# Autonomous-Drone-Racing-Lab/Efficient-Path-Planner

Hardware: AMD Instinct MI355X
Metric: validity checks/sec + full plan ms/track, 1/2/4/8 MI355X vs CPU ref (higher is better)
Workload: dtype f64; 1 GPU; C2: 1 track, 8 gates, 64 OBBs, 1,048,576 sampled states per step; obbs=64, can_pass_gate=False, parallelism=replicas x1 (independent samplers), process_group=solo, launch=hip graph of the K steps

## Files before the change

### efficient-path-planner_amd/csrc/collision_common.h

```cpp
#pragma once
#include <hip/hip_runtime.h>

#include <algorithm>
#include <cstdlib>
#include <mutex>
#include <set>
#include <string>

#include "epp_internal.h"

namespace epp {
SmallWorld small_world(const epp_world* w);
epp_status note_record_reader(const epp_world* w, const SmallWorld& sw, hipStream_t st);

constexpr int64_t kSmallStates = 4096;
constexpr int64_t kSmallMotions = 1024;
constexpr int kSmallMaxObbs = 256;
bool small_states(const SmallWorld& sw, int64_t n);
bool small_motions(const SmallWorld& sw, int64_t n);
epp_status launch_states_small(const SmallWorld& sw, bool mindist, const double* xyz, int64_t n, int32_t can_pass,
                               double md, uint8_t* valid, int32_t* compact_idx, int64_t* n_valid, hipStream_t st,
                               uint32_t* done = nullptr, uint32_t seq = 0);
epp_status launch_motions_small(const SmallWorld& sw, int32_t mode, const double* s1, const double* s2, int64_t n,
                                int32_t can_pass, uint8_t* valid, hipStream_t st, uint32_t* done = nullptr,
// ... 341 lines not shown
    const double tx = fillb ? rr[F_HX] : rr[F_HX] + r, ty = fillb ? rr[F_HY] : rr[F_HY] + r,
                 tz = fillb ? rr[F_HZ] : rr[F_HZ] + r;
    clip(c * ax + sn * ay, c * d[0] + sn * d[1], -tx, tx);
    clip(c * ay - sn * ax, c * d[1] - sn * d[0], -ty, ty);
    clip(ps[2] - rr[F_CZ], d[2], -tz, tz);
    int k0 = 33, k1 = 0;
    if (t0 <= t1) {
        k0 = max(1, (int)ceil(32.0 * t0));
        k1 = min(32, (int)floor(32.0 * t1));
    }
    bool hit = false;
    for (int k = k0; k <= k1 && !hit; ++k) {
        const double t = (double)k / 32.0;
        const double qx = ps[0] + (pe[0] - ps[0]) * t;
        const double qy = ps[1] + (pe[1] - ps[1]) * t;
        const double qz = ps[2] + (pe[2] - ps[2]) * t;
        hit = rec_hit<false>(rr, rg, ro, qx, qy, qz, cp, 0.0);
    }
    return hit;
}

template <bool MINDIST>
__device__ __forceinline__ bool states_exact_rec(const unsigned char* sbase, uint32_t lists_off, uint32_t ids_off,
                                                 double rg, double ro, double px, double py, double pz, uint32_t cls,
                                                 int can_pass, double md) {
    const double* recs = reinterpret_cast<const double*>(sbase);
    const uint32_t h = reinterpret_cast<const uint32_t*>(sbase + lists_off)[cls];
    const uint16_t* ids = reinterpret_cast<const uint16_t*>(sbase + ids_off) + (h >> 12);
    const uint32_t cnt = h & 4095u;
    bool hit = false;
    for (uint32_t j = 0; j < cnt; ++j)
        hit |= rec_hit<MINDIST>(recs + (size_t)ids[j] * kRecDoubles, rg, ro, px, py, pz, can_pass != 0, md);
    return hit;
}


__device__ __forceinline__ bool rec_ray_hit(const double* rec, const double s[3], const double e[3], double r) {
    double f[kRecDoubles];
#pragma unroll
    for (int k = 0; k <= F_HZ; ++k) f[k] = rec[k];
    f[R_META] = rec[R_META];
    const uint32_t m = (uint32_t)__double_as_longlong(f[R_META]);
    const bool fill = (m & META_FILLING) != 0u;
    const double c = f[F_COS], sn = f[F_SIN];
    const double cx = f[F_CX], cy = f[F_CY], cz = f[F_CZ];
    const double h[3] = {f[F_HX], f[F_HY], f[F_HZ]};
    const double ph0 = fill ? h[0] : h[0] + r, ph1 = fill ? h[1] : h[1] + r, ph2 = fill ? h[2] : h[2] + r;
    double ls[3], ld[3];
    bool end_hit;
    {
        const double dx = s[0] - cx, dy = s[1] - cy, dz = s[2] - cz;
        ls[0] = c * dx + sn * dy;
        ls[1] = c * dy - sn * dx;
        ls[2] = dz;
        const double ex = e[0] - cx, ey = e[1] - cy, ez = e[2] - cz;
// ... 90 lines not shown
```

### efficient-path-planner_amd/csrc/epp_internal.h

```cpp
#pragma once
#include <math.h>
#include <stdint.h>

#include <mutex>
#include <shared_mutex>
#include <string>
#include <vector>

#include <hip/hip_runtime_api.h>

#include "epp.h"

namespace epp {
epp_status generate_trajectory_into(const double* wp, int32_t n_wp, const double* times, double v_max,
                                    double a_max, double dt, double t0, const double v0[3], const double a0[3],
                                    double* (*alloc)(void*, int64_t), void* ctx, int64_t* n_rows);
struct FusedCheck {
    const epp_world* world;
    const double* xyz;
    int64_t n;
    double min_distance;
    uint8_t* valid;
};
epp_status check_and_generate_into(const FusedCheck* chk, const double* wp, int32_t n_wp, const double* times,
// ... 44 lines not shown
           o_query = 0, o_ids32 = 0, o_rows32 = 0, o_rows16 = 0, o_ev = 0, o_mark = 0, o_map = 0, o_nstat = 0,
           o_need = 0, dev_bytes = 0;
    size_t h_seg = 0, h_hdr = 0, h_slot = 0, h_rows = 0, h_need = 0, h_done = 0, host_bytes = 0;
    int32_t done_n = 0;
};
PlanBatchLayout plan_batch_layout(int32_t S, int64_t ns, int32_t k, PlanSeg* segs);
void plan_batch_trace_print();
epp_status plan_batch_launch(const epp_world* world, int32_t can_pass_gate, const double lo[3], const double hi[3],
                             const PlanBatchLayout& L, void* dev, void* host, uint32_t seq, void* stream);
}

namespace epp {

enum Field : int {
    F_LOX = 0, F_LOY, F_LOZ, F_HIX, F_HIY, F_HIZ,
    F_CX, F_CY, F_CZ,
    F_COS, F_SIN,
    F_HX, F_HY, F_HZ,
    EPP_NF
};

constexpr int kRecDoubles = 17;
constexpr int R_META = 16;

constexpr size_t kListMaxLen = 4095;
constexpr size_t kStageBudget = 64 * 1024;

constexpr uint32_t META_FILLING = 1u;
constexpr uint32_t META_GATE = 2u;
constexpr int kMaxGridAxis = 255;

struct WorldView {
    const unsigned char* blob;
    uint32_t blob_bytes;
    int32_t n_obb;
    int32_t n_pad;
    int32_t nx, ny, nz;
    uint32_t front_bytes;
    uint32_t off_cell_mask;
    uint32_t off_cell_start;
    uint32_t off_cell_obb;
    uint32_t off_meta;
    uint32_t off_soa;
    double gx0, gy0, gz0;
    double gx1, gy1, gz1;
    double icx, icy, icz;
    float ofx, ofy, ofz;
    float i4x, i4y, i4z;
    float limx, limy, limz;
    float fmaxx, fmaxy, fmaxz;
    double r_gate, r_obst;
    uint32_t off_aos;
    uint32_t off_lists;
    uint32_t off_ids;
    uint32_t n_lists;
    uint32_t off_bitmap;
    uint32_t bm_words;
    uint32_t off_cls8;
    uint32_t cls8_bytes;
    int32_t bnx, bny, bnz;
    float bofx, bofy, bofz;
    float bix, biy, biz;
    uint32_t off_slab;
    int32_t slab_n;
    int32_t slab_log;
    int32_t slab_w;
    int32_t tile_n;
    uint32_t tile_words;
    float sofx, sofy, sofz;
    float six, siy, siz;
};

constexpr int kSlabMaxWords = 32;
constexpr size_t kSlabBudget = 40 * 1024;
constexpr size_t kSlabBudgetMax = 64 * 1024;
constexpr size_t kMotionsLdsFree = 150 * 1024 - 16 * (256 * 4 + 64);
#if defined(__HIPCC__)
// ... 88 lines not shown
```

### efficient-path-planner_amd/csrc/states.hip

```cpp
#include "collision_common.h"

namespace epp {
namespace {

template <int STAGE, bool MINDIST, bool ALIGNED>
__global__ __launch_bounds__(kBlock) void k_states(WorldView w, const double* __restrict__ xyz,
                                                   int64_t n, int can_pass, double md,
                                                   uint8_t* __restrict__ valid,
                                                   int32_t* __restrict__ compact_idx,
                                                   unsigned long long* __restrict__ n_valid,
                                                   uint32_t stage_bytes) {
    extern __shared__ __attribute__((aligned(16))) unsigned char lds[];
    const int lane = threadIdx.x & 63;
    const int64_t groups = n / 4;
    const int64_t stride = (int64_t)gridDim.x * kBlock;
    auto load = [&](int64_t grp, double (&dst)[12]) {
        grp = grp < groups ? grp : groups - 1;
        if (ALIGNED) {
            const double2* q = reinterpret_cast<const double2*>(xyz + 12 * grp);
#pragma unroll
            for (int k = 0; k < 6; ++k) {
                const double2 t = q[k];
                dst[2 * k] = t.x;
                dst[2 * k + 1] = t.y;
// ... 155 lines not shown
    extern __shared__ __attribute__((aligned(16))) unsigned char lds_blob[];
    const int lane = threadIdx.x & 63;
    const int wave = __builtin_amdgcn_readfirstlane(threadIdx.x >> 6);
    BmParams bp;
    bp.cls = (gptr_u16)(wv->blob + wv->off_bitmap);
    bp.ox = wv->bofx; bp.oy = wv->bofy; bp.oz = wv->bofz;
    bp.ix = wv->bix; bp.iy = wv->biy; bp.iz = wv->biz;
    bp.nx = (uint32_t)wv->bnx; bp.ny = (uint32_t)wv->bny; bp.nz = (uint32_t)wv->bnz;
    bp.sentinel = wv->bm_words;
    const uint32_t stride = gridDim.x * kBlock4;
    uint32_t it = blockIdx.x * kBlock4 + threadIdx.x;
    double v[6];
    auto load = [&](uint32_t i) {
        i = i < items ? i : items - 1;
        const double2* p = reinterpret_cast<const double2*>(xyz) + 3 * (size_t)i;
#pragma unroll
        for (int k = 0; k < 3; ++k) {
            const double2 t = p[k];
            v[2 * k] = t.x;
            v[2 * k + 1] = t.y;
        }
    };
    if (items > 0) load(it);
    const uint32_t lists_off = wv->off_lists - wv->off_aos, ids_off = wv->off_ids - wv->off_aos;
    const double rg = wv->r_gate, ro = wv->r_obst;
    const unsigned char* xbase;
    if (STAGE) {
        stage_copy(lds_blob, wv->blob + wv->off_aos, stage_bytes, kBlock4);
        xbase = lds_blob;
    } else {
        xbase = wv->blob + wv->off_aos;
    }
    for (uint32_t i0 = blockIdx.x * kBlock4; i0 < items; i0 += stride, it += stride) {
        if (i0 != blockIdx.x * kBlock4) load(it);
        const bool live = it < items;
        const uint32_t c0 = bp.cls[cls_index(bp, v[0], v[1], v[2])];
        const uint32_t c1 = bp.cls[cls_index(bp, v[3], v[4], v[5])];
        const bool n0 = live & (c0 != 0u), n1 = live & (c1 != 0u);
        const unsigned long long b0 = __ballot(n0), b1 = __ballot(n1);
        const uint32_t t0 = (uint32_t)__popcll(b0), tw = t0 + (uint32_t)__popcll(b1);
        if (lane == 0) q.wcnt[wave] = tw;
        __syncthreads();
        uint32_t off = 0, T = 0;
        for (int w = 0; w < wave; ++w) off += q.wcnt[w];
        T = off;
        for (int w = wave; w < kBlock4 / 64; ++w) T += q.wcnt[w];
        uint32_t hits = 0;
        if (T > 0) {
            const uint32_t p0 = off + lanes_below(b0), p1 = off + t0 + lanes_below(b1);
            if (n0) {
                q.x[p0] = v[0];
                q.y[p0] = v[1];
                q.z[p0] = v[2];
                q.cls[p0] = (uint16_t)c0;
            }
            if (n1) {
                q.x[p1] = v[3];
                q.y[p1] = v[4];
                q.z[p1] = v[5];
                q.cls[p1] = (uint16_t)c1;
            }
            __syncthreads();
            for (uint32_t e = threadIdx.x; e < T; e += kBlock4)
                q.hit[e] = states_exact_rec<MINDIST>(xbase, lists_off, ids_off, rg, ro, q.x[e], q.y[e], q.z[e], q.cls[e],
                                                     can_pass, md)
                               ? 1
                               : 0;
            __syncthreads();
            hits = (n0 && q.hit[p0] ? 1u : 0u) | (n1 && q.hit[p1] ? 2u : 0u);
        }
        const uint32_t fl = live ? (~hits & 3u) : 0u;
        if (live) *reinterpret_cast<uint16_t*>(valid + 2 * (size_t)it) = (uint16_t)((fl & 1u) | ((fl & 2u) << 7));
        if (COMPACT) {
            const uint32_t c = (uint32_t)__popc(fl);
            uint32_t ctot;
            const uint32_t cex = wave_excl_scan(c, lane, ctot);
            unsigned long long wbase = 0;
            if (lane == 0 && ctot) wbase = atomicAdd(n_valid, (unsigned long long)ctot);
            wbase = __shfl(wbase, 0, 64);
            uint64_t p = wbase + cex;
            if (fl & 1u) compact_idx[p++] = (int32_t)(2 * (size_t)it);
            if (fl & 2u) compact_idx[p] = (int32_t)(2 * (size_t)it + 1);
        }
    }
    if (STAGE && items == 0) __syncthreads();
    if (blockIdx.x == 0 && threadIdx.x == 0 && (n & 1)) {
        const int64_t i = n - 1;
        const double px = xyz[3 * i], py = xyz[3 * i + 1], pz = xyz[3 * i + 2];
        const uint32_t c = bp.cls[cls_index(bp, px, py, pz)];
        const bool ok = !(c != 0u && states_exact_rec<MINDIST>(xbase, lists_off, ids_off, rg, ro, px, py, pz, c, can_pass, md));
        valid[i] = ok ? 1 : 0;
        if (COMPACT && ok) compact_idx[atomicAdd(n_valid, 1ull)] = (int32_t)i;
    }
}

struct WaveQueue5 {
    double x[64], y[64], z[64];
    uint32_t hdr[64];
};
template <int BLOCK>
constexpr uint32_t queue5_bytes() { return (BLOCK / 64) * sizeof(WaveQueue5); }

__device__ __forceinline__ uint32_t cell_axis5(double p, float off, float inv, uint32_t nm1) {
    const float f = fmaf((float)p, inv, off);
    int i;
    asm("v_cvt_i32_f32 %0, %1" : "=v"(i) : "v"(f));
    return min((uint32_t)i, nm1);
}
__device__ __forceinline__ uint32_t mad_u24(uint32_t a, uint32_t b, uint32_t c) {
    uint32_t r;
    asm("v_mad_u32_u24 %0, %1, %2, %3" : "=v"(r) : "v"(a), "s"(b), "v"(c));
    return r;
}
// ... 2 lines not shown
}

#ifdef EPP_STATES_TL
constexpr int kTlWaves = 1 << 16;
constexpr int kTlWords = 8;
__device__ unsigned long long g_states_tl[kTlWaves][kTlWords];
#define EPP_STL(k)                                                                                  \
    do {                                                                                            \
        const int w_ = (int)((blockIdx.x * BLOCK + threadIdx.x) >> 6);                             \
        const unsigned long long t_ = __builtin_amdgcn_s_memrealtime();                             \
        if ((threadIdx.x & 63) == 0 && w_ < kTlWaves) g_states_tl[w_][k] = t_;                      \
    } while (0)
#else
#define EPP_STL(k) \
    do {           \
    } while (0)
#endif

struct V5Args {
    uint32_t lists_off, ids_off;
    uint32_t cls_off, cls_nz_off;
    uint32_t nx, ny, nz;
    float ox, oy, oz, ix, iy, iz;
    double rg, ro;
};

template <bool MINDIST, bool COMPACT, int BLOCK, bool PREFETCH, int SPL, bool C8, int SC>
__global__ __launch_bounds__(BLOCK) __attribute__((amdgpu_waves_per_eu(BLOCK == 512 && !PREFETCH ? 5 : BLOCK / 256)))
void k_states_v5(const unsigned char* stage_src, const double* xyz,
                                                     int64_t groups, uint32_t stage_bytes, int can_pass,
                                                     int64_t n, double md, uint8_t* __restrict__ valid,
                                                     int32_t* __restrict__ compact_idx,
                                                     unsigned long long* __restrict__ n_valid, V5Args wa) {
    __shared__ WaveQueue5 queues[BLOCK / 64];
    extern __shared__ __attribute__((aligned(16))) unsigned char lds_blob[];
    const int lane = threadIdx.x & 63;
    EPP_STL(0);
    WaveQueue5* qu = &queues[threadIdx.x >> 6];
    const int64_t stride = (int64_t)gridDim.x * BLOCK;
    const int64_t gfirst = (int64_t)blockIdx.x * BLOCK;
    int64_t g = gfirst + threadIdx.x;
    constexpr int NV = 3 * SPL;
    double va[NV], vb[NV];
    const double* xyzb = groups > 0 ? xyz : reinterpret_cast<const double*>(stage_src);
    auto load = [&](int64_t grp, double (&dst)[NV]) {
        grp = grp < groups ? grp : groups - 1;
        grp = grp < 0 ? 0 : grp;
// ... 11 lines not shown
    const uint32_t n16 = stage_bytes / 16u;
#if defined(__HIP_DEVICE_COMPILE__)
    typedef const __attribute__((address_space(1))) u32x4* gptr_stage;
    const gptr_stage ssrc = (gptr_stage)stage_src;
#else
    const u32x4* ssrc = reinterpret_cast<const u32x4*>(stage_src);
#endif
#pragma unroll
    for (int i = 0; i < kStageChunks; ++i) {
        const uint32_t o = (uint32_t)(i * BLOCK) + threadIdx.x;
        stg[i] = ssrc[o < n16 ? o : n16 - 1u];
    }
    load(g, va);
#pragma unroll
    for (int i = 0; i < kStageChunks; ++i) {
        const uint32_t o = (uint32_t)(i * BLOCK) + threadIdx.x;
        *reinterpret_cast<u32x4*>(lds_blob + 16u * (o < n16 ? o : n16)) = stg[i];
    }
    const uint32_t lists_off = wa.lists_off, ids_off = wa.ids_off;
    const unsigned char* cls_base = lds_blob + wa.cls_off;
    [[maybe_unused]] const unsigned char* cls_nz = lds_blob + wa.cls_nz_off;
    const uint32_t* hdrs = reinterpret_cast<const uint32_t*>(lds_blob + lists_off);
    const uint16_t* ids_all = reinterpret_cast<const uint16_t*>(lds_blob + ids_off);
    const double* recs = reinterpret_cast<const double*>(lds_blob);
    const float ox = wa.ox, oy = wa.oy, oz = wa.oz, ix = wa.ix, iy = wa.iy, iz = wa.iz;
    const uint32_t nx = wa.nx, ny = wa.ny, nz = wa.nz;
    const double rg = wa.rg, ro = wa.ro;
    __syncthreads();
    EPP_STL(1);
    auto cell_of = [&](double px, double py, double pz) -> uint32_t {
        const uint32_t cx = cell_axis5(px, ox, ix, nx - 1), cy = cell_axis5(py, oy, iy, ny - 1),
                       cz = cell_axis5(pz, oz, iz, nz - 1);
        return mad_u24(mad_u24(cz, ny, cy), nx, cx);
    };
    auto classes_of = [&](const auto& idx, auto& c, auto& occ) {
        constexpr int N = (int)(sizeof(idx) / sizeof(idx[0]));
        if (C8) {
            uint64_t wd[N];
            uint32_t rank[N];
#pragma unroll
            for (int k = 0; k < N; ++k) wd[k] = reinterpret_cast<const uint64_t*>(cls_base)[idx[k] >> 5];
#pragma unroll
            for (int k = 0; k < N; ++k) {
                const uint32_t m = (uint32_t)wd[k], sh = idx[k] & 31u;
                rank[k] = (uint32_t)(wd[k] >> 32) + (uint32_t)__popc(m & ((1u << sh) - 1u));
                occ[k] = (m >> sh) & 1u;
            }
#pragma unroll
            for (int k = 0; k < N; ++k) c[k] = (uint32_t)cls_nz[rank[k]];
#pragma unroll
            for (int k = 0; k < N; ++k) c[k] = occ[k] ? c[k] : 0u;
            return;
// ... 58 lines not shown
                    }
                }
                wave_lds_sync();
                const uint32_t tq = min(total - r0, 64u);
                const bool act = (uint32_t)lane < tq;
                const uint32_t hq = act ? qu->hdr[lane] : 0u;
                const uint32_t cnt = hq & 4095u, first = hq >> 12;
                uint32_t ptot;
                const uint32_t poff = wave_excl_scan(cnt, lane, ptot);
#ifdef EPP_STATES_TL
                tl_needy += tq;
                tl_pairs += ptot;
#endif
                bool hit_e = false;
                if (ptot <= 128u) {
                    uint32_t ln = (uint32_t)lane;
                    asm volatile("" : "+v"(ln));
                    const uint32_t head = (ln << 21) + (first - poff + ((1u << 21) + 128u));
                    const bool own0 = act & (poff < 64u);
                    const uint32_t head0 = (uint32_t)__builtin_amdgcn_readfirstlane((int)head);
                    const uint32_t h0 = dpp_incl_max(lane_scatter(own0 ? poff : 0u, own0 ? head : head0));
                    auto test = [&](uint32_t h, uint32_t q) {
                        const uint32_t e = (h >> 21) - 1u;
                        return q < ptot &&
                               rec_hit<MINDIST>(recs + (size_t)ids_all[(h & 0x1FFFFFu) + q - 128u] * kRecDoubles, rg, ro,
                                                qu->x[e], qu->y[e], qu->z[e], can_pass != 0, md);
                    };
                    unsigned long long m1 = 0ull;
                    uint32_t h1 = 0u;
                    if (ptot > 64u) {
                        const uint32_t plast = (uint32_t)__builtin_amdgcn_readlane((int)poff, (int)(tq - 1u));
                        const uint32_t hlast = (uint32_t)__builtin_amdgcn_readlane((int)head, (int)(tq - 1u));
                        const bool own1 = act & (poff >= 64u);
                        const uint32_t carry = (uint32_t)__builtin_amdgcn_readlane((int)h0, 63);
                        h1 = max(dpp_incl_max(lane_scatter(own1 ? poff : plast,
                                                           own1 ? head : (plast >= 64u ? hlast : 0u))),
                                 carry);
                    }
                    const unsigned long long m0 = __builtin_amdgcn_ballot_w64(test(h0, (uint32_t)lane));
                    if (ptot > 64u) m1 = __builtin_amdgcn_ballot_w64(test(h1, 64u + (uint32_t)lane));
                    auto bits = [](unsigned long long m, uint32_t from, uint32_t len) {
                        const unsigned long long msk = len >= 64u ? ~0ull : ((1ull << len) - 1ull);
                        return ((m >> from) & msk) != 0ull;
                    };
                    const uint32_t end = poff + cnt;
                    const bool lo = poff < 64u && bits(m0, poff, min(end, 64u) - poff);
                    const bool hi = end > 64u && bits(m1, poff > 64u ? poff - 64u : 0u, end - max(poff, 64u));
                    hit_e = act && (lo || hi);
                } else if (act) {
                    const double* rc = reinterpret_cast<const double*>(lds_blob);
                    const uint16_t* idl = reinterpret_cast<const uint16_t*>(lds_blob + ids_off) + first;
                    const double px = qu->x[lane], py = qu->y[lane], pz = qu->z[lane];
                    for (uint32_t j = 0; j < cnt; ++j)
                        hit_e |= rec_hit<MINDIST>(rc + (size_t)idl[j] * kRecDoubles, rg, ro, px, py, pz, can_pass != 0,
                                                  md);
                }
                const unsigned long long hm = __builtin_amdgcn_ballot_w64(hit_e);
#pragma unroll
                for (int k = 0; k < SPL; ++k) {
                    const uint32_t slot = pos[k] - r0;
                    if (needy[k] && slot < 64u && ((hm >> slot) & 1ull)) hits |= 1u << k;
                }
                wave_lds_sync();
            }
        }
        EPP_STL(4);
        const uint32_t fl = live ? (~hits & ((1u << SPL) - 1u)) : 0u;
        if (live) {
            if (SPL == 4) {
                *reinterpret_cast<uint32_t*>(valid + 4 * gg) =
                    (fl & 1u) | ((fl & 2u) << 7) | ((fl & 4u) << 14) | ((fl & 8u) << 21);
            } else {
                unsigned long long w = 0ull;
#pragma unroll
                for (int k = 0; k < SPL; ++k) w |= (unsigned long long)((fl >> k) & 1u) << (8 * k);
                *reinterpret_cast<unsigned long long*>(valid + SPL * gg) = w;
            }
        }
// ... 21 lines not shown
    } else {
        for (int64_t g0 = gfirst; g0 < groups; g0 += stride, g += stride) {
            if (g0 != gfirst) load(g, va);
            process(g, va);
        }
    }
#ifdef EPP_STATES_TL
    EPP_STL(5);
    if (lane == 0) {
        unsigned hw;
        asm volatile("s_getreg_b32 %0, hwreg(HW_REG_HW_ID)" : "=s"(hw));
        const int w_ = (int)((blockIdx.x * BLOCK + threadIdx.x) >> 6);
        if (w_ < kTlWaves)
            g_states_tl[w_][6] = hw | ((unsigned long long)min(tl_needy, 65535u) << 32) |
                                 ((unsigned long long)min(tl_pairs, 65535u) << 48);
    }
#endif
    if (blockIdx.x == 0 && threadIdx.x < (int)(n - SPL * groups)) {
        const int64_t i = SPL * groups + threadIdx.x;
        const double px = xyz[3 * i], py = xyz[3 * i + 1], pz = xyz[3 * i + 2];
        const uint32_t cell[1] = {cell_of(px, py, pz)};
        uint32_t c[1], occ[1];
        classes_of(cell, c, occ);
        const bool ok = !(occ[0] != 0u && states_exact_rec<MINDIST>(lds_blob, lists_off, ids_off, rg, ro, px, py, pz, c[0],
                                                              can_pass, md));
        valid[i] = ok ? 1 : 0;
        if (COMPACT && ok) compact_idx[atomicAdd(n_valid, 1ull)] = (int32_t)i;
    }
}

enum class StatesKernel { V5, V4, Generic };
StatesKernel forced_kernel() {
    const char* v = std::getenv("EPP_STATES_KERNEL");
    if (!v || !*v) return StatesKernel::V5;
    const std::string k(v);
    return k == "generic" ? StatesKernel::Generic : k == "v4" ? StatesKernel::V4 : StatesKernel::V5;
}

uint32_t v5_staged(const WorldView& w) {
    return (w.off_cls8 ? ((w.off_cls8 + w.cls8_bytes + 15u) & ~15u) : w.blob_bytes) - w.off_aos;
}
V5Args v5_args(const WorldView& w) {
    V5Args a{};
    a.lists_off = w.off_lists - w.off_aos;
    a.ids_off = w.off_ids - w.off_aos;
    a.cls_off = (w.off_cls8 ? w.off_cls8 : w.off_bitmap) - w.off_aos;
    a.cls_nz_off = a.cls_off + ((w.bm_words + 1u + 31u) >> 5) * 8u;
    a.nx = (uint32_t)w.bnx; a.ny = (uint32_t)w.bny; a.nz = (uint32_t)w.bnz;
    a.ox = w.bofx; a.oy = w.bofy; a.oz = w.bofz;
    a.ix = w.bix; a.iy = w.biy; a.iz = w.biz;
    a.rg = w.r_gate; a.ro = w.r_obst;
    return a;
}
constexpr uint32_t kV5DummyBytes = 96;
bool v5_fits(const WorldView& w) {
    const uint32_t sb = v5_staged(w);
    return sb <= kStageBudget && sb + 16u + queue5_bytes<1024>() <= 160u * 1024u;
}

struct V5Shape {
    int64_t gN;
    int bs, grid;
    bool pf;
};
V5Shape v5_shape(int64_t n, uint32_t sb) {
    V5Shape r{};
    const int64_t cus = cu_count();
    r.gN = n / 4;
    const int forced = env_int("EPP_V5_BLOCK", 0);
    if (forced == 256 && 4u * (sb + 16u + queue5_bytes<256>()) <= 160u * 1024u && r.gN <= 4 * cus * 256) {
        r.bs = 256;
        r.grid = (int)std::max<int64_t>(1, (r.gN + 255) / 256);
        r.pf = false;
        return r;
    }
    const bool two = forced == 0 && 2u * (sb + 16u + queue5_bytes<512>()) <= 160u * 1024u && r.gN <= 2 * cus * 512;
    if (two) {
        r.bs = 512;
        r.grid = (int)std::max<int64_t>(1, (r.gN + 511) / 512);
        r.pf = false;
        return r;
    }
    const bool single = r.gN <= cus * 1024;
    r.bs = forced == 512 ? 512 : forced == 1024 ? 1024 : (single ? 1024 : 512);
    r.grid = (int)std::max<int64_t>(1, std::min<int64_t>((r.gN + r.bs - 1) / r.bs, cus));
    r.pf = r.gN > (int64_t)r.grid * r.bs;
    return r;
}

bool v4_stage(const WorldView& w) { return (w.off_bitmap - w.off_aos) + sizeof(StateQueue4) <= 160u * 1024u; }
int v4_grid(const WorldView& w, int64_t n) {
    const int64_t items = std::max<int64_t>(1, n / 2);
    const int64_t need = (items + kBlock4 - 1) / kBlock4;
    const uint32_t lds = sizeof(StateQueue4) + (v4_stage(w) ? w.off_bitmap - w.off_aos : 0u);
    const int per_cu = std::max(1, std::min<int>(3, (int)((160u * 1024u) / lds)));
    const int64_t cap = (int64_t)cu_count() * per_cu;
    return (int)std::max<int64_t>(1, std::min(need, cap));
}

template <bool MINDIST>
epp_status launch_states(const WorldView& w, const WorldView* dw, const double* xyz, int64_t n, int32_t can_pass,
                         double md, uint8_t* valid, int32_t* compact_idx, int64_t* n_valid, void* stream) {
    hipStream_t st = (hipStream_t)stream;
    auto nv = reinterpret_cast<unsigned long long*>(n_valid);
    const char* what = MINDIST ? "epp_check_states_mindist" : "epp_check_states";
    const StatesKernel want = forced_kernel();
    const bool x16 = (reinterpret_cast<uintptr_t>(xyz) & 15) == 0;
    if (want == StatesKernel::V5 && v5_fits(w) && x16 && (reinterpret_cast<uintptr_t>(valid) & 3) == 0 &&
        (n >= 4 || w.blob_bytes - w.off_aos >= kV5DummyBytes)) {
        const uint32_t sb = v5_staged(w);
        V5Shape sh = v5_shape(n, sb);
        if (sh.bs == 256 && compact_idx) {
            sh.bs = 512;
            sh.grid = (int)std::max<int64_t>(1, (sh.gN + 511) / 512);
        }
        const uint32_t dyn = sb + 16u;
        const unsigned char* src = w.blob + w.off_aos;
        const V5Args wa = v5_args(w);
#define EPP_LAUNCH_V5S(C, B, P, C8, SC)                                                                              \
    do {                                                                                                             \
        allow_lds(k_states_v5<MINDIST, C, B, P, 4, C8, SC>, queue5_bytes<B>());                                      \
        hipLaunchKernelGGL((k_states_v5<MINDIST, C, B, P, 4, C8, SC>), dim3(sh.grid), dim3(B), dyn, st, src, xyz,   \
                           sh.gN, sb, can_pass, n, md, valid, compact_idx, nv, wa);                                  \
    } while (0)
        const bool half_stage = sb <= (uint32_t)kStageBudget / 2;
#define EPP_LAUNCH_V5C(C, B, P, C8)                                                              \
    do {                                                                                         \
        if (sb <= (uint32_t)B * 16u) EPP_LAUNCH_V5S(C, B, P, C8, 1);                              \
        else if (sb <= (uint32_t)B * 32u) EPP_LAUNCH_V5S(C, B, P, C8, 2);                         \
        else if (sb <= (uint32_t)B * 48u) EPP_LAUNCH_V5S(C, B, P, C8, 3);                         \
        else if (half_stage) EPP_LAUNCH_V5S(C, B, P, C8, (int)(kStageBudget / 2 / (B * 16)));    \
        else EPP_LAUNCH_V5S(C, B, P, C8, (int)(kStageBudget / (B * 16)));                        \
    } while (0)
#define EPP_LAUNCH_V5(C, B, P)                                 \
    do {                                                       \
        if (w.off_cls8) EPP_LAUNCH_V5C(C, B, P, true);          \
        else EPP_LAUNCH_V5C(C, B, P, false);                    \
    } while (0)
#define EPP_LAUNCH_V5B(B)                                \
    do {                                                 \
        if (sh.pf) {                                     \
            if (compact_idx) EPP_LAUNCH_V5(true, B, true);  \
            else EPP_LAUNCH_V5(false, B, true);          \
        } else {                                         \
            if (compact_idx) EPP_LAUNCH_V5(true, B, false); \
            else EPP_LAUNCH_V5(false, B, false);         \
        }                                                \
    } while (0)
        if (sh.bs == 256) EPP_LAUNCH_V5(false, 256, false);
        else if (sh.bs == 512) EPP_LAUNCH_V5B(512);
        else EPP_LAUNCH_V5B(1024);
#undef EPP_LAUNCH_V5B
#undef EPP_LAUNCH_V5
#undef EPP_LAUNCH_V5C
#undef EPP_LAUNCH_V5S
        return launch_error(what);
    }
    if (want != StatesKernel::Generic && x16 && (reinterpret_cast<uintptr_t>(valid) & 1) == 0 &&
        n / 2 < 0xFFFFFFFFll) {
        const uint32_t sb = w.off_bitmap - w.off_aos;
        const bool stg = v4_stage(w);
        const int g4 = v4_grid(w, n);
        const uint32_t items = (uint32_t)(n / 2);
#define EPP_LAUNCH_V4(S, C)                                                                                      \
    do {                                                                                                         \
        allow_lds(k_states_v4<MINDIST, S, C>, sizeof(StateQueue4));                                              \
        hipLaunchKernelGGL((k_states_v4<MINDIST, S, C>), dim3(g4), dim3(kBlock4), S ? sb : 0, st, dw, xyz, items, n, \
                           can_pass, md, valid, compact_idx, nv, sb);                                            \
    } while (0)
        if (compact_idx) {
            if (stg) EPP_LAUNCH_V4(true, true);
            else EPP_LAUNCH_V4(false, true);
        } else {
            if (stg) EPP_LAUNCH_V4(true, false);
            else EPP_LAUNCH_V4(false, false);
        }
#undef EPP_LAUNCH_V4
        return launch_error(what);
    }
    const bool aligned = (x16 & ((reinterpret_cast<uintptr_t>(valid) & 3) == 0));
    const bool lds = w.front_bytes + kScratchBytes <= kLdsBudget;
    const uint32_t stage = !lds ? 0u : (w.blob_bytes <= 40u * 1024u ? w.blob_bytes : w.front_bytes);
    const uint32_t shm = kScratchBytes + stage;
// ... 77 lines not shown
```

### efficient-path-planner_amd/csrc/world_index.cpp

```cpp
#include <hip/hip_runtime.h>

#include <algorithm>
#include <chrono>
#include <cmath>
#include <cstdlib>
#include <cstring>
#include <mutex>
#include <new>
#include <string>
#include <vector>

#include "epp_internal.h"

namespace epp {
namespace {

void compute_aabb(const epp_obb& o, double inflate, double lo[3], double hi[3]) {
    static const double sx[8] = {-1, 1, 1, -1, -1, 1, 1, -1};
    static const double sy[8] = {-1, -1, 1, 1, -1, -1, 1, 1};
    static const double sz[8] = {-1, -1, -1, -1, 1, 1, 1, 1};
    for (int j = 0; j < 8; ++j) {
        const double c0 = sx[j] * o.half[0], c1 = sy[j] * o.half[1], c2 = sz[j] * o.half[2];
        for (int i = 0; i < 3; ++i) {
            const double g =
// ... 288 lines not shown
        v.bnx = bd[0]; v.bny = bd[1]; v.bnz = bd[2];
        v.bofx = bo[0]; v.bofy = bo[1]; v.bofz = bo[2];
        v.bix = bi[0]; v.biy = bi[1]; v.biz = bi[2];
        v.bm_words = (uint32_t)cells;
        v.n_lists = (uint32_t)hdr.size();
        break;
    }
    const size_t n_entries = cell_start[ncell];
    const size_t off_mask = 0;
    const size_t off_cs = align16(off_mask + mask.size() * 8);
    const size_t front = align16(off_cs + cell_start.size() * 4);
    const size_t off_co = front;
    const size_t off_meta = align16(off_co + n_entries * 2);
    const size_t off_soa = align16(off_meta + meta.size() * 4);
    std::vector<double> aos((size_t)n * kRecDoubles, 0.0);
    for (int i = 0; i < n; ++i) {
        double* r = &aos[(size_t)i * kRecDoubles];
        const double* f = soa.data();
        const int fields[14] = {F_LOX, F_LOY, F_LOZ, F_HIX, F_HIY, F_HIZ, F_CX, F_CY, F_CZ, F_COS, F_SIN, F_HX, F_HY, F_HZ};
        for (int k = 0; k < 14; ++k) r[k] = f[(size_t)fields[k] * n_pad + i];
        uint64_t m = meta[i];
        std::memcpy(&r[R_META], &m, 8);
    }
    const size_t off_aos = align16(off_soa + soa.size() * sizeof(double));
    const size_t off_lists = align16(off_aos + aos.size() * sizeof(double));
    const size_t off_ids = off_lists + hdr.size() * 4;
    const bool c8 = hdr.size() <= 256;
    const size_t off_c8 = align16(off_ids + flat.size() * 2);
    std::vector<uint64_t> cwords;
    std::vector<uint8_t> cnz;
    if (c8) {
        cwords.assign((cls.size() + 31) / 32, 0ull);
        for (size_t w = 0; w < cwords.size(); ++w) {
            uint32_t m = 0;
            const uint64_t before = cnz.size();
            for (size_t j = 0; j < 32 && 32 * w + j < cls.size(); ++j)
                if (cls[32 * w + j]) {
                    m |= 1u << j;
                    cnz.push_back((uint8_t)cls[32 * w + j]);
                }
            cwords[w] = (uint64_t)m | (before << 32);
        }
    }
    const size_t c8_bytes = c8 ? cwords.size() * 8 + cnz.size() : 0;
    const size_t off_bm = c8 ? align16(off_c8 + c8_bytes) : off_c8;
    std::vector<uint32_t> slab;
    int S = 0, SL = 0, W = 0, T = 0;
    uint32_t tw = 0;
// ... 82 lines not shown
            }
    }
    v.slab_n = S;
    v.slab_log = SL;
    v.slab_w = W;
    v.tile_n = T;
    v.tile_words = tw;
    v.sofx = so[0]; v.sofy = so[1]; v.sofz = so[2];
    v.six = si[0]; v.siy = si[1]; v.siz = si[2];
    const size_t off_slab = align16(off_bm + cls.size() * 2);
    const size_t total = align16(off_slab + slab.size() * 4);
    if (total > 0xFFFFFFFFull) {
        set_error("epp_world: index too large");
        return false;
    }
    hw.blob.assign(total, '\0');
    char* b = &hw.blob[0];
    std::memcpy(b + off_mask, mask.data(), mask.size() * 8);
    std::memcpy(b + off_cs, cell_start.data(), cell_start.size() * 4);
    if (n_entries) std::memcpy(b + off_co, cell_obb.data(), n_entries * 2);
    std::memcpy(b + off_meta, meta.data(), meta.size() * 4);
    std::memcpy(b + off_soa, soa.data(), soa.size() * sizeof(double));
    if (!aos.empty()) std::memcpy(b + off_aos, aos.data(), aos.size() * sizeof(double));
    std::memcpy(b + off_lists, hdr.data(), hdr.size() * 4);
    if (!flat.empty()) std::memcpy(b + off_ids, flat.data(), flat.size() * 2);
    v.off_ids = (uint32_t)off_ids;
    v.off_aos = (uint32_t)off_aos;
    std::memcpy(b + off_bm, cls.data(), cls.size() * 2);
    if (!slab.empty()) std::memcpy(b + off_slab, slab.data(), slab.size() * 4);
    v.off_slab = (uint32_t)off_slab;
    if (c8) {
        std::memcpy(b + off_c8, cwords.data(), cwords.size() * 8);
        if (!cnz.empty()) std::memcpy(b + off_c8 + cwords.size() * 8, cnz.data(), cnz.size());
    }
    v.off_cls8 = c8 ? (uint32_t)off_c8 : 0u;
    v.cls8_bytes = (uint32_t)c8_bytes;
    v.off_lists = (uint32_t)off_lists;
    v.off_bitmap = (uint32_t)off_bm;
    v.blob_bytes = (uint32_t)total;
    v.front_bytes = (uint32_t)front;
    v.off_cell_mask = (uint32_t)off_mask;
    v.off_cell_start = (uint32_t)off_cs;
    v.off_cell_obb = (uint32_t)off_co;
    v.off_meta = (uint32_t)off_meta;
    v.off_soa = (uint32_t)off_soa;
    return true;
}

bool upload(HostWorld& hw) {
    const size_t bytes = hw.blob.size();
// ... 289 lines not shown
    for (int r = 0; r < reps; ++r)
        if (!epp::build_blob(hw, obbs, n)) return EPP_ERR_UNSUPPORTED;
    const auto t1 = std::chrono::steady_clock::now();
    out[0] = std::chrono::duration<double, std::micro>(t1 - t0).count() / reps;
    out[1] = hw.view.blob_bytes;
    out[2] = hw.view.tile_n;
    out[3] = hw.view.tile_words;
    out[4] = hw.view.slab_w;
    out[5] = hw.view.slab_n;
    return EPP_OK;
}

extern "C" epp_status epp_dbg_class_layout(const epp_obb* obbs, int32_t n, double r_gate, double r_obst,
                                           int64_t out[12]) {
    if (!out || n < 0 || (n > 0 && !obbs)) return EPP_ERR_INVALID_ARGUMENT;
    epp::HostWorld hw;
    hw.r_gate = r_gate;
    hw.r_obst = r_obst;
    if (!epp::build_blob(hw, obbs, n)) return EPP_ERR_UNSUPPORTED;
    const epp::WorldView& v = hw.view;
    const int64_t vals[12] = {v.off_aos, v.off_lists, v.off_ids, v.off_cls8, v.off_bitmap, v.blob_bytes, v.n_lists,
                              v.bm_words, v.bnx, v.bny, v.bnz,
                              (int64_t)((v.off_cls8 ? ((v.off_cls8 + v.cls8_bytes + 15u) & ~15u) : v.blob_bytes) -
                                        v.off_aos)};
    for (int k = 0; k < 12; ++k) out[k] = vals[k];
    return EPP_OK;
}

extern "C" int64_t epp_dbg_check_sparse_classes(const epp_obb* obbs, int32_t n, double r_gate, double r_obst) {
    if (n < 0 || (n > 0 && !obbs)) return -2;
    epp::HostWorld hw;
    hw.r_gate = r_gate;
    hw.r_obst = r_obst;
    if (!epp::build_blob(hw, obbs, n)) return -2;
    const epp::WorldView& v = hw.view;
    if (!v.off_cls8) return -1;
    const unsigned char* b = reinterpret_cast<const unsigned char*>(hw.blob.data());
    const uint16_t* cls = reinterpret_cast<const uint16_t*>(b + v.off_bitmap);
    const unsigned char* base = b + v.off_cls8;
    const unsigned char* nz = base + ((v.bm_words + 1u + 31u) >> 5) * 8u;
    int64_t bad = 0;
    for (uint32_t idx = 0; idx <= v.bm_words; ++idx) {
        uint64_t wd;
        std::memcpy(&wd, base + (size_t)(idx >> 5) * 8, 8);
        const uint32_t m = (uint32_t)wd, sh = idx & 31u;
        const uint32_t rank = (uint32_t)(wd >> 32) + (uint32_t)__builtin_popcount(m & ((1u << sh) - 1u));
        const uint32_t c = ((m >> sh) & 1u) ? (uint32_t)nz[rank] : 0u;
        bad += c != (uint32_t)cls[idx];
// ... 4 lines not shown
```

Before: 147.9 billion state validity checks/s.

## Add precomputed point-test records with swizzled LDS layout for state checks

Builds a second per-OBB record array with 16 doubles per box. The radius-inflated half-extents are precomputed, and the records are stored in XOR-swizzled 16-byte chunks so LDS reads avoid bank conflicts. The filling flag is packed into the high bit of each list id. The non-mindist V5 path stages only these point records, lists and class data into LDS and runs a branch-light point_rec_hit, which removes the 17-double record load and the radius arithmetic from each check. This enlarges the blob and the V4 staging footprint, and the V5 path is restricted to worlds where the id flag fits.

```diff
diff --git a/efficient-path-planner_amd/csrc/collision_common.h b/efficient-path-planner_amd/csrc/collision_common.h
--- a/efficient-path-planner_amd/csrc/collision_common.h
+++ b/efficient-path-planner_amd/csrc/collision_common.h
@@ -387,15 +387,43 @@
 
 template <bool MINDIST>
 __device__ __forceinline__ bool states_exact_rec(const unsigned char* sbase, uint32_t lists_off, uint32_t ids_off,
-                                                 double rg, double ro, double px, double py, double pz, uint32_t cls,
-                                                 int can_pass, double md) {
+                                                 uint32_t id_mask, double rg, double ro, double px, double py,
+                                                 double pz, uint32_t cls, int can_pass, double md) {
     const double* recs = reinterpret_cast<const double*>(sbase);
     const uint32_t h = reinterpret_cast<const uint32_t*>(sbase + lists_off)[cls];
     const uint16_t* ids = reinterpret_cast<const uint16_t*>(sbase + ids_off) + (h >> 12);
     const uint32_t cnt = h & 4095u;
     bool hit = false;
     for (uint32_t j = 0; j < cnt; ++j)
-        hit |= rec_hit<MINDIST>(recs + (size_t)ids[j] * kRecDoubles, rg, ro, px, py, pz, can_pass != 0, md);
+        hit |= rec_hit<MINDIST>(recs + (size_t)(ids[j] & id_mask) * kRecDoubles, rg, ro, px, py, pz, can_pass != 0, md);
+    return hit;
+}
+
+__device__ __forceinline__ bool point_rec_hit(const unsigned char* pts, uint32_t ide, double px, double py, double pz,
+                                              bool can_pass) {
+    typedef double f64x2 __attribute__((ext_vector_type(2)));
+    const uint32_t i = ide & (kIdFill - 1u);
+    f64x2 q[7];
+#pragma unroll
+    for (uint32_t k = 0; k < 7; ++k) q[k] = *reinterpret_cast<const f64x2*>(pts + pt_chunk_off(i, k));
+    const double lox = q[0].x, loy = q[0].y, loz = q[1].x, hix = q[1].y, hiy = q[2].x, hiz = q[2].y;
+    const double cx = q[3].x, cy = q[3].y, cz = q[4].x, c = q[4].y, s = q[5].x;
+    const double tx = q[5].y, ty = q[6].x, tz = q[6].y;
+    const bool in = (lox < px) & (px < hix) & (loy < py) & (py < hiy) & (loz < pz) & (pz < hiz);
+    const bool skip = ((ide & kIdFill) != 0u) & can_pass;
+    const double dx = px - cx, dy = py - cy, dz = pz - cz;
+    const double lx = c * dx + s * dy;
+    const double ly = c * dy - s * dx;
+    return in & !skip & (fabs(lx) <= tx) & (fabs(ly) <= ty) & (fabs(dz) <= tz);
+}
+
+__device__ __forceinline__ bool states_exact_pt(const unsigned char* sbase, uint32_t lists_off, uint32_t ids_off,
+                                                double px, double py, double pz, uint32_t cls, int can_pass) {
+    const uint32_t h = reinterpret_cast<const uint32_t*>(sbase + lists_off)[cls];
+    const uint16_t* ids = reinterpret_cast<const uint16_t*>(sbase + ids_off) + (h >> 12);
+    const uint32_t cnt = h & 4095u;
+    bool hit = false;
+    for (uint32_t j = 0; j < cnt; ++j) hit |= point_rec_hit(sbase, ids[j], px, py, pz, can_pass != 0);
     return hit;
 }
 
diff --git a/efficient-path-planner_amd/csrc/epp_internal.h b/efficient-path-planner_amd/csrc/epp_internal.h
--- a/efficient-path-planner_amd/csrc/epp_internal.h
+++ b/efficient-path-planner_amd/csrc/epp_internal.h
@@ -90,6 +90,14 @@
 
 constexpr int kRecDoubles = 17;
 constexpr int R_META = 16;
+
+constexpr int kPtDoubles = 16;
+constexpr int P_TX = F_HX, P_TY = F_HY, P_TZ = F_HZ;
+#if defined(__HIPCC__)
+__host__ __device__
+#endif
+constexpr uint32_t pt_chunk_off(uint32_t i, uint32_t c) { return (i << 7) + ((c ^ ((i >> 1) & 7u)) << 4); }
+constexpr uint32_t kIdFill = 0x8000u;
 
 constexpr size_t kListMaxLen = 4095;
 constexpr size_t kStageBudget = 64 * 1024;
@@ -119,8 +127,10 @@
     float fmaxx, fmaxy, fmaxz;
     double r_gate, r_obst;
     uint32_t off_aos;
+    uint32_t off_pt;
     uint32_t off_lists;
     uint32_t off_ids;
+    uint32_t id_mask;
     uint32_t n_lists;
     uint32_t off_bitmap;
     uint32_t bm_words;
diff --git a/efficient-path-planner_amd/csrc/states.hip b/efficient-path-planner_amd/csrc/states.hip
--- a/efficient-path-planner_amd/csrc/states.hip
+++ b/efficient-path-planner_amd/csrc/states.hip
@@ -201,11 +201,15 @@
         }
     };
     if (items > 0) load(it);
-    const uint32_t lists_off = wv->off_lists - wv->off_aos, ids_off = wv->off_ids - wv->off_aos;
+    const uint32_t rec_bytes = wv->off_pt - wv->off_aos;
+    const uint32_t lists_off = STAGE ? rec_bytes : wv->off_lists - wv->off_aos;
+    const uint32_t ids_off = lists_off + (wv->off_ids - wv->off_lists);
+    const uint32_t id_mask = wv->id_mask;
     const double rg = wv->r_gate, ro = wv->r_obst;
     const unsigned char* xbase;
     if (STAGE) {
-        stage_copy(lds_blob, wv->blob + wv->off_aos, stage_bytes, kBlock4);
+        stage_copy(lds_blob, wv->blob + wv->off_aos, rec_bytes, kBlock4);
+        stage_copy(lds_blob + rec_bytes, wv->blob + wv->off_lists, stage_bytes - rec_bytes, kBlock4);
         xbase = lds_blob;
     } else {
         xbase = wv->blob + wv->off_aos;
@@ -241,7 +245,7 @@
             }
             __syncthreads();
             for (uint32_t e = threadIdx.x; e < T; e += kBlock4)
-                q.hit[e] = states_exact_rec<MINDIST>(xbase, lists_off, ids_off, rg, ro, q.x[e], q.y[e], q.z[e], q.cls[e],
+                q.hit[e] = states_exact_rec<MINDIST>(xbase, lists_off, ids_off, id_mask, rg, ro, q.x[e], q.y[e], q.z[e], q.cls[e],
                                                      can_pass, md)
                                ? 1
                                : 0;
@@ -267,7 +271,7 @@
         const int64_t i = n - 1;
         const double px = xyz[3 * i], py = xyz[3 * i + 1], pz = xyz[3 * i + 2];
         const uint32_t c = bp.cls[cls_index(bp, px, py, pz)];
-        const bool ok = !(c != 0u && states_exact_rec<MINDIST>(xbase, lists_off, ids_off, rg, ro, px, py, pz, c, can_pass, md));
+        const bool ok = !(c != 0u && states_exact_rec<MINDIST>(xbase, lists_off, ids_off, id_mask, rg, ro, px, py, pz, c, can_pass, md));
         valid[i] = ok ? 1 : 0;
         if (COMPACT && ok) compact_idx[atomicAdd(n_valid, 1ull)] = (int32_t)i;
     }
@@ -316,7 +320,6 @@
     uint32_t cls_off, cls_nz_off;
     uint32_t nx, ny, nz;
     float ox, oy, oz, ix, iy, iz;
-    double rg, ro;
 };
 
 template <bool MINDIST, bool COMPACT, int BLOCK, bool PREFETCH, int SPL, bool C8, int SC>
@@ -374,12 +377,17 @@
     [[maybe_unused]] const unsigned char* cls_nz = lds_blob + wa.cls_nz_off;
     const uint32_t* hdrs = reinterpret_cast<const uint32_t*>(lds_blob + lists_off);
     const uint16_t* ids_all = reinterpret_cast<const uint16_t*>(lds_blob + ids_off);
-    const double* recs = reinterpret_cast<const double*>(lds_blob);
     const float ox = wa.ox, oy = wa.oy, oz = wa.oz, ix = wa.ix, iy = wa.iy, iz = wa.iz;
     const uint32_t nx = wa.nx, ny = wa.ny, nz = wa.nz;
-    const double rg = wa.rg, ro = wa.ro;
     __syncthreads();
     EPP_STL(1);
+    auto hit_of = [&](uint32_t ide, double px, double py, double pz) -> bool {
+        if constexpr (MINDIST)
+            return rec_hit<true>(reinterpret_cast<const double*>(lds_blob) + (size_t)(ide & (kIdFill - 1u)) * kRecDoubles,
+                                 0.0, 0.0, px, py, pz, false, md);
+        else
+            return point_rec_hit(lds_blob, ide, px, py, pz, can_pass != 0);
+    };
     auto cell_of = [&](double px, double py, double pz) -> uint32_t {
         const uint32_t cx = cell_axis5(px, ox, ix, nx - 1), cy = cell_axis5(py, oy, iy, ny - 1),
                        cz = cell_axis5(pz, oz, iz, nz - 1);
@@ -484,9 +492,7 @@
                     const uint32_t h0 = dpp_incl_max(lane_scatter(own0 ? poff : 0u, own0 ? head : head0));
                     auto test = [&](uint32_t h, uint32_t q) {
                         const uint32_t e = (h >> 21) - 1u;
-                        return q < ptot &&
-                               rec_hit<MINDIST>(recs + (size_t)ids_all[(h & 0x1FFFFFu) + q - 128u] * kRecDoubles, rg, ro,
-                                                qu->x[e], qu->y[e], qu->z[e], can_pass != 0, md);
+                        return q < ptot && hit_of(ids_all[(h & 0x1FFFFFu) + q - 128u], qu->x[e], qu->y[e], qu->z[e]);
                     };
                     unsigned long long m1 = 0ull;
                     uint32_t h1 = 0u;
@@ -510,12 +516,9 @@
                     const bool hi = end > 64u && bits(m1, poff > 64u ? poff - 64u : 0u, end - max(poff, 64u));
                     hit_e = act && (lo || hi);
                 } else if (act) {
-                    const double* rc = reinterpret_cast<const double*>(lds_blob);
                     const uint16_t* idl = reinterpret_cast<const uint16_t*>(lds_blob + ids_off) + first;
                     const double px = qu->x[lane], py = qu->y[lane], pz = qu->z[lane];
-                    for (uint32_t j = 0; j < cnt; ++j)
-                        hit_e |= rec_hit<MINDIST>(rc + (size_t)idl[j] * kRecDoubles, rg, ro, px, py, pz, can_pass != 0,
-                                                  md);
+                    for (uint32_t j = 0; j < cnt; ++j) hit_e |= hit_of(idl[j], px, py, pz);
                 }
                 const unsigned long long hm = __builtin_amdgcn_ballot_w64(hit_e);
 #pragma unroll
@@ -583,8 +586,14 @@
         const uint32_t cell[1] = {cell_of(px, py, pz)};
         uint32_t c[1], occ[1];
         classes_of(cell, c, occ);
-        const bool ok = !(occ[0] != 0u && states_exact_rec<MINDIST>(lds_blob, lists_off, ids_off, rg, ro, px, py, pz, c[0],
-                                                              can_pass, md));
+        bool hit = false;
+        if (occ[0] != 0u) {
+            if constexpr (MINDIST)
+                hit = states_exact_rec<true>(lds_blob, lists_off, ids_off, kIdFill - 1u, 0.0, 0.0, px, py, pz, c[0], 0, md);
+            else
+                hit = states_exact_pt(lds_blob, lists_off, ids_off, px, py, pz, c[0], can_pass);
+        }
+        const bool ok = !hit;
         valid[i] = ok ? 1 : 0;
         if (COMPACT && ok) compact_idx[atomicAdd(n_valid, 1ull)] = (int32_t)i;
     }
@@ -598,25 +607,26 @@
     return k == "generic" ? StatesKernel::Generic : k == "v4" ? StatesKernel::V4 : StatesKernel::V5;
 }
 
-uint32_t v5_staged(const WorldView& w) {
-    return (w.off_cls8 ? ((w.off_cls8 + w.cls8_bytes + 15u) & ~15u) : w.blob_bytes) - w.off_aos;
-}
-V5Args v5_args(const WorldView& w) {
+uint32_t v5_start(const WorldView& w, bool mindist) { return mindist ? w.off_aos : w.off_pt; }
+uint32_t v5_staged(const WorldView& w, bool mindist) {
+    return (w.off_cls8 ? ((w.off_cls8 + w.cls8_bytes + 15u) & ~15u) : w.blob_bytes) - v5_start(w, mindist);
+}
+V5Args v5_args(const WorldView& w, bool mindist) {
     V5Args a{};
-    a.lists_off = w.off_lists - w.off_aos;
-    a.ids_off = w.off_ids - w.off_aos;
-    a.cls_off = (w.off_cls8 ? w.off_cls8 : w.off_bitmap) - w.off_aos;
+    const uint32_t start = v5_start(w, mindist);
+    a.lists_off = w.off_lists - start;
+    a.ids_off = w.off_ids - start;
+    a.cls_off = (w.off_cls8 ? w.off_cls8 : w.off_bitmap) - start;
     a.cls_nz_off = a.cls_off + ((w.bm_words + 1u + 31u) >> 5) * 8u;
     a.nx = (uint32_t)w.bnx; a.ny = (uint32_t)w.bny; a.nz = (uint32_t)w.bnz;
     a.ox = w.bofx; a.oy = w.bofy; a.oz = w.bofz;
     a.ix = w.bix; a.iy = w.biy; a.iz = w.biz;
-    a.rg = w.r_gate; a.ro = w.r_obst;
     return a;
 }
 constexpr uint32_t kV5DummyBytes = 96;
-bool v5_fits(const WorldView& w) {
-    const uint32_t sb = v5_staged(w);
-    return sb <= kStageBudget && sb + 16u + queue5_bytes<1024>() <= 160u * 1024u;
+bool v5_fits(const WorldView& w, bool mindist) {
+    const uint32_t sb = v5_staged(w, mindist);
+    return sb <= kStageBudget && sb + 16u + queue5_bytes<1024>() <= 160u * 1024u && w.id_mask == kIdFill - 1u;
 }
 
 struct V5Shape {
@@ -649,11 +659,12 @@
     return r;
 }
 
-bool v4_stage(const WorldView& w) { return (w.off_bitmap - w.off_aos) + sizeof(StateQueue4) <= 160u * 1024u; }
+uint32_t v4_staged(const WorldView& w) { return (w.off_pt - w.off_aos) + (w.off_bitmap - w.off_lists); }
+bool v4_stage(const WorldView& w) { return v4_staged(w) + sizeof(StateQueue4) <= 160u * 1024u; }
 int v4_grid(const WorldView& w, int64_t n) {
     const int64_t items = std::max<int64_t>(1, n / 2);
     const int64_t need = (items + kBlock4 - 1) / kBlock4;
-    const uint32_t lds = sizeof(StateQueue4) + (v4_stage(w) ? w.off_bitmap - w.off_aos : 0u);
+    const uint32_t lds = sizeof(StateQueue4) + (v4_stage(w) ? v4_staged(w) : 0u);
     const int per_cu = std::max(1, std::min<int>(3, (int)((160u * 1024u) / lds)));
     const int64_t cap = (int64_t)cu_count() * per_cu;
     return (int)std::max<int64_t>(1, std::min(need, cap));
@@ -667,17 +678,17 @@
     const char* what = MINDIST ? "epp_check_states_mindist" : "epp_check_states";
     const StatesKernel want = forced_kernel();
     const bool x16 = (reinterpret_cast<uintptr_t>(xyz) & 15) == 0;
-    if (want == StatesKernel::V5 && v5_fits(w) && x16 && (reinterpret_cast<uintptr_t>(valid) & 3) == 0 &&
-        (n >= 4 || w.blob_bytes - w.off_aos >= kV5DummyBytes)) {
-        const uint32_t sb = v5_staged(w);
+    if (want == StatesKernel::V5 && v5_fits(w, MINDIST) && x16 && (reinterpret_cast<uintptr_t>(valid) & 3) == 0 &&
+        (n >= 4 || w.blob_bytes - v5_start(w, MINDIST) >= kV5DummyBytes)) {
+        const uint32_t sb = v5_staged(w, MINDIST);
         V5Shape sh = v5_shape(n, sb);
         if (sh.bs == 256 && compact_idx) {
             sh.bs = 512;
             sh.grid = (int)std::max<int64_t>(1, (sh.gN + 511) / 512);
         }
         const uint32_t dyn = sb + 16u;
-        const unsigned char* src = w.blob + w.off_aos;
-        const V5Args wa = v5_args(w);
+        const unsigned char* src = w.blob + v5_start(w, MINDIST);
+        const V5Args wa = v5_args(w, MINDIST);
 #define EPP_LAUNCH_V5S(C, B, P, C8, SC)                                                                              \
     do {                                                                                                             \
         allow_lds(k_states_v5<MINDIST, C, B, P, 4, C8, SC>, queue5_bytes<B>());                                      \
@@ -719,7 +730,7 @@
     }
     if (want != StatesKernel::Generic && x16 && (reinterpret_cast<uintptr_t>(valid) & 1) == 0 &&
         n / 2 < 0xFFFFFFFFll) {
-        const uint32_t sb = w.off_bitmap - w.off_aos;
+        const uint32_t sb = v4_staged(w);
         const bool stg = v4_stage(w);
         const int g4 = v4_grid(w, n);
         const uint32_t items = (uint32_t)(n / 2);
diff --git a/efficient-path-planner_amd/csrc/world_index.cpp b/efficient-path-planner_amd/csrc/world_index.cpp
--- a/efficient-path-planner_amd/csrc/world_index.cpp
+++ b/efficient-path-planner_amd/csrc/world_index.cpp
@@ -334,8 +334,26 @@
         uint64_t m = meta[i];
         std::memcpy(&r[R_META], &m, 8);
     }
+    const bool id_flags = n <= 32768;
+    std::vector<double> pts((size_t)n * kPtDoubles, 0.0);
+    for (int i = 0; i < n; ++i) {
+        const double* a = &aos[(size_t)i * kRecDoubles];
+        const bool fill = (meta[i] & META_FILLING) != 0u;
+        const double r = (meta[i] & META_GATE) ? hw.r_gate : hw.r_obst;
+        double f[kPtDoubles] = {};
+        for (int k = 0; k <= F_SIN; ++k) f[k] = a[k];
+        const double ix = a[F_HX] + r, iy = a[F_HY] + r, iz = a[F_HZ] + r;
+        f[P_TX] = fill ? a[F_HX] : ix;
+        f[P_TY] = fill ? a[F_HY] : iy;
+        f[P_TZ] = fill ? a[F_HZ] : iz;
+        char* dst = reinterpret_cast<char*>(pts.data());
+        for (uint32_t c = 0; c < 8; ++c) std::memcpy(dst + pt_chunk_off((uint32_t)i, c), &f[2 * c], 16);
+    }
+    if (id_flags)
+        for (auto& id : flat) id = (uint16_t)(id | ((meta[id] & META_FILLING) ? kIdFill : 0u));
     const size_t off_aos = align16(off_soa + soa.size() * sizeof(double));
-    const size_t off_lists = align16(off_aos + aos.size() * sizeof(double));
+    const size_t off_pt = align16(off_aos + aos.size() * sizeof(double));
+    const size_t off_lists = off_pt + pts.size() * sizeof(double);
     const size_t off_ids = off_lists + hdr.size() * 4;
     const bool c8 = hdr.size() <= 256;
     const size_t off_c8 = align16(off_ids + flat.size() * 2);
@@ -464,10 +482,13 @@
     std::memcpy(b + off_meta, meta.data(), meta.size() * 4);
     std::memcpy(b + off_soa, soa.data(), soa.size() * sizeof(double));
     if (!aos.empty()) std::memcpy(b + off_aos, aos.data(), aos.size() * sizeof(double));
+    if (!pts.empty()) std::memcpy(b + off_pt, pts.data(), pts.size() * sizeof(double));
     std::memcpy(b + off_lists, hdr.data(), hdr.size() * 4);
     if (!flat.empty()) std::memcpy(b + off_ids, flat.data(), flat.size() * 2);
     v.off_ids = (uint32_t)off_ids;
+    v.id_mask = id_flags ? kIdFill - 1u : 0xFFFFu;
     v.off_aos = (uint32_t)off_aos;
+    v.off_pt = (uint32_t)off_pt;
     std::memcpy(b + off_bm, cls.data(), cls.size() * 2);
     if (!slab.empty()) std::memcpy(b + off_slab, slab.data(), slab.size() * 4);
     v.off_slab = (uint32_t)off_slab;
@@ -803,8 +824,35 @@
     const int64_t vals[12] = {v.off_aos, v.off_lists, v.off_ids, v.off_cls8, v.off_bitmap, v.blob_bytes, v.n_lists,
                               v.bm_words, v.bnx, v.bny, v.bnz,
                               (int64_t)((v.off_cls8 ? ((v.off_cls8 + v.cls8_bytes + 15u) & ~15u) : v.blob_bytes) -
-                                        v.off_aos)};
+                                        v.off_pt)};
     for (int k = 0; k < 12; ++k) out[k] = vals[k];
+    return EPP_OK;
+}
+
+extern "C" epp_status epp_dbg_point_records(const epp_obb* obbs, int32_t n, double r_gate, double r_obst,
+                                            double* recs17, double* pt16, uint16_t* ids, int64_t ids_cap,
+                                            int64_t out[6]) {
+    if (!out || n < 0 || (n > 0 && (!obbs || !recs17 || !pt16)) || ids_cap < 0 || (ids_cap > 0 && !ids))
+        return EPP_ERR_INVALID_ARGUMENT;
+    epp::HostWorld hw;
+    hw.r_gate = r_gate;
+    hw.r_obst = r_obst;
+    if (!epp::build_blob(hw, obbs, n)) return EPP_ERR_UNSUPPORTED;
+    const epp::WorldView& v = hw.view;
+    const char* b = hw.blob.data();
+    int64_t n_ids = 0;
+    for (uint32_t l = 0; l < v.n_lists; ++l) {
+        uint32_t h;
+        std::memcpy(&h, b + v.off_lists + 4 * (size_t)l, 4);
+        n_ids = std::max<int64_t>(n_ids, (int64_t)(h >> 12) + (h & 4095u));
+    }
+    if (n > 0) std::memcpy(recs17, b + v.off_aos, (size_t)n * epp::kRecDoubles * 8);
+    for (int i = 0; i < n; ++i)
+        for (uint32_t c = 0; c < 8; ++c)
+            std::memcpy(pt16 + (size_t)i * epp::kPtDoubles + 2 * c, b + v.off_pt + epp::pt_chunk_off((uint32_t)i, c), 16);
+    if (ids_cap > 0) std::memcpy(ids, b + v.off_ids, (size_t)std::min<int64_t>(ids_cap, n_ids) * 2);
+    const int64_t vals[6] = {v.off_aos, v.off_pt, v.off_lists, v.off_ids, n_ids, v.id_mask};
+    for (int k = 0; k < 6; ++k) out[k] = vals[k];
     return EPP_OK;
 }
 
```

Measured after the change: 152.2 billion state validity checks/s (median of 6 runs). 2.9% higher.
